# Rhizomatica/mercury

Hardware: AMD Instinct MI355X
Metric: RX frames/s (mode 8, max 50 LDPC iters) (higher is better)
Workload: dtype f64

## Files before the change

include/mercury_gpu.h:

```cpp
#ifndef MERCURY_GPU_H
#define MERCURY_GPU_H

#include <stddef.h>
#include <stdint.h>

#ifdef __cplusplus
extern "C" {
#endif

#define MGPU_OK 0
#define MGPU_ERR_ARG 1
#define MGPU_ERR_DEVICE 2
#define MGPU_ERR_TABLES 3
#define MGPU_ERR_UNSUPPORTED 4

#define MGPU_DEC_GBF 0
#define MGPU_DEC_SPA 1
#define MGPU_DEC_MINSUM 2
#define MGPU_DEC_SPA_FAST 3

#define MGPU_EST_ZF 0
#define MGPU_EST_LS 1

typedef struct mgpu_ctx mgpu_ctx;
// ... 130 lines not shown
    long long crc_ok_frames;
} mgpu_error_rate;
int mgpu_baseband_test_esn0(mgpu_ctx* ctx, const double* esn0_db, int npoints, long long frames_per_point, uint64_t seed, uint64_t frame0,
                            int channel, mgpu_error_rate* out);

int mgpu_passband_to_baseband(mgpu_ctx* ctx, const double* passband , int W, int in_size,
                              const double* carrier_hz , int filter, const int* start , int count,
                              int decimation, double* out_c128 );
int mgpu_time_sync_preamble(mgpu_ctx* ctx, const double* baseband_interp_c128 , int W, int size, int step,
                            int location_to_return, int nTrials_max, int* delay , double* correlation );
int mgpu_freq_sync(mgpu_ctx* ctx, const double* baseband_c128 , int W, int stride, double* freq_offset_hz );
int mgpu_time_sync_mfsk(mgpu_ctx* ctx, const double* baseband_interp_c128 , int W, int size, int search_start_symb,
                        int* delay );
int mgpu_detect_ack_pattern(mgpu_ctx* ctx, const double* baseband_interp_c128 , int W, int size, int pattern,
                            double* metric , int* matched );
int mgpu_detect_ack_pattern_from_passband(mgpu_ctx* ctx, const double* passband , int W, int size, double carrier_hz,
                                          int pattern, double* metric , int* matched );
int mgpu_last_sync_kernel_ms(mgpu_ctx* ctx, float* ms);

int mgpu_enable_timing(mgpu_ctx* ctx, int on);
int mgpu_kernel_ms_avg(mgpu_ctx* ctx, float ms[2], int* n_launches);
int mgpu_decoder_hard_frames(mgpu_ctx* ctx, long long* frames);
int mgpu_host_path_last(mgpu_ctx* ctx, int* chunk_frames, int* n_chunks, float* fill_ms, float* drain_ms, float* total_ms);
int mgpu_last_kernel_ms(mgpu_ctx* ctx, float ms[2]);

int mgpu_debug_mfsk_sync(mgpu_ctx* ctx, const double* energy, int W, int nslots, int size, const int* search_start, int variant, int* delay);
int mgpu_debug_p2b_variant(int variant);
int mgpu_debug_span_energy(mgpu_ctx* ctx, const double* bb, int W, int size, const int* wv, const int* off, int n, int len, int variant, double* sum,
                           int* cnt);
int mgpu_debug_spa_math(mgpu_ctx* ctx, const double* in, int n, double* tanh_out, double* atanh_out);
int mgpu_debug_select_peak(mgpu_ctx* ctx, const double* cand_vals, int n, int ncand_max, const int* ncand, const int* size, const int* loc, int step,
                           int nTrials_max, int* delay, double* corr);

int mgpu_debug_occupancy(mgpu_ctx* ctx, int which);

int mgpu_debug_tsync_metric(mgpu_ctx* ctx, const double* baseband_interp, int W, int size, int step, int variant, const int* start, const int* sub_size,
                            double* vals);

int mgpu_debug_glibc_trig(mgpu_ctx* ctx, const double* in, int n, double* atan_out, double* sin_out, double* cos_out);

#ifdef __cplusplus
}
#endif
#endif
```

mercury_amd/csrc/ctx.hpp:

```cpp
#pragma once
#include <hip/hip_runtime.h>

#include <functional>
#include <memory>
#include <stdexcept>
#include <string>
#include <type_traits>
#include <utility>
#include <vector>

#include <cmath>
#include "../../include/mercury_gpu.h"
#include "../../include/mercury_rxloop.h"
#include "../../include/mercury_channel.h"
#include "device_tables.h"
#include "tables.hpp"

extern "C" const unsigned char mgpu_ldpc_blob[];
extern "C" const unsigned long mgpu_ldpc_blob_size;

extern "C" size_t mgpu_frontend_lds_bytes(int G, int nPilots, int nBits, int threads);
extern "C" size_t mgpu_spa_lds_bytes(int E, int N);
extern "C" size_t mgpu_gbf_lds_bytes(int N);
extern "C" size_t mgpu_spa_fast_lds_bytes(int Sg, int N);
extern "C" size_t mgpu_txgen_lds_bytes(int G);

extern "C" __global__ void mgpu_frontend_kernel(MgpuDev, const double*, int, float*, float*, float*, double*, MgpuTapsDev);
extern "C" __global__ void mgpu_frontend_kernel_t1024(MgpuDev, const double*, int, float*, float*, float*, double*, MgpuTapsDev);
extern "C" __global__ void mgpu_mfsk_frontend_kernel_m32(MgpuDev, const double*, int, int, float*, float*, float*, MgpuTapsDev);
extern "C" __global__ void mgpu_mfsk_frontend_kernel_m16x2(MgpuDev, const double*, int, int, float*, float*, float*, MgpuTapsDev);
extern "C" int mgpu_mfsk_syms_per_block();
extern "C" __global__ void mgpu_slot_energy_kernel(const double*, int, int, int, const double*, double*);
extern "C" __global__ void mgpu_mfsk_sync_kernel(const double*, int, int, MgpuMfskSync, const int*, int*);
extern "C" __global__ void mgpu_zf_snr_kernel(MgpuDev, const uint8_t*, const double*, int, MgpuStatsDev*, double*);
extern "C" size_t mgpu_zfsnr_lds_bytes(int nData);
extern "C" __global__ void mgpu_p2b_kernel(const double*, int, const double*, const int*, int, int, int, const double*, int, double, double, double*, const int*, const double*, const int*, int);
extern "C" __global__ void mgpu_p2b_slide_d1_kernel(const double*, int, const double*, const int*, int, int, const double*, double, double, double*, const int*, const double*, const int*, int);
extern "C" __global__ void mgpu_p2b_slide_d4_kernel(const double*, int, const double*, const int*, int, int, const double*, double, double, double*, const int*, const double*, const int*, int);
extern "C" __global__ void mgpu_p2b_slide_d1_sincos_kernel(const double*, int, const double*, const int*, int, int, const double*, double, double, double*, const int*, const double*, const int*, int);
extern "C" __global__ void mgpu_p2b_slide_d4_sincos_kernel(const double*, int, const double*, const int*, int, int, const double*, double, double, double*, const int*, const double*, const int*, int);
struct MgpuKernelGeometry { int outputs_per_block, threads, lds_bytes; };
struct MgpuStreamGeometry { int step, ngi, nfft, pre, K, ring; };
extern "C" MgpuKernelGeometry mgpu_p2b_slide_geometry(int decim);
extern "C" __global__ void mgpu_tsync_metric_kernel(const double*, int, const int*, const int*, const int*, int, int, int, int, int, double*);
extern "C" __global__ void mgpu_tsync_metric_dense_kernel(const double*, int, const int*, const int*, const int*, int, int, int, int, int, double*);
extern "C" int mgpu_tsync_coarse_threads();
extern "C" __global__ void mgpu_tsync_metric_stream_kernel(const double*, int, const int*, const int*, const int*, int, double*, int, int, int);
extern "C" MgpuStreamGeometry mgpu_tsync_stream_geometry();
extern "C" __global__ void mgpu_tsync_metric_fine_kernel_r4(const double*, int, const int*, const int*, const int*, int, int, int, int, double*);
extern "C" __global__ void mgpu_tsync_metric_fine_kernel_r8(const double*, int, const int*, const int*, const int*, int, int, int, int, double*);
extern "C" MgpuKernelGeometry mgpu_tsync_fine_geometry(int R);
// ... 58 lines not shown
    using DevBuf::DevBuf;
    operator T*() const { return static_cast<T*>(p); }
};
template <typename H, hipError_t (*Destroy)(H)> struct Handle {
    H h = nullptr;
    Handle() = default;
    Handle(Handle&& o) noexcept { std::swap(h, o.h); }
    Handle& operator=(Handle&& o) noexcept { std::swap(h, o.h); return *this; }
    ~Handle() { if (h) (void)Destroy(h); }
    operator H() const { return h; }
};
using Stream = Handle<hipStream_t, hipStreamDestroy>;
using Event = Handle<hipEvent_t, hipEventDestroy>;
using GraphExec = Handle<hipGraphExec_t, hipGraphExecDestroy>;
using PinnedBuf = Handle<void*, hipHostFree>;

template <typename T>
DevArray<T> upload(const std::vector<T>& v) {
    DevArray<T> d(v.size() * sizeof(T) + 16);
    HIPCK(hipMemcpy(d.p, v.data(), v.size() * sizeof(T), hipMemcpyHostToDevice));
    return d;
}

struct Workspace;
struct TxState;
struct Release { void operator()(Workspace*) const; void operator()(TxState*) const; };

}
using namespace mgpu_detail;

struct mgpu_ctx {
    mgpu_config cfg{};
    mgpu::ModeTables tab;
    MgpuDev dev{};
    LdpcDev ldev{};
    std::vector<DevBuf> tables;
    std::string err;
    int max_batch = 0;
    int numa_node = -1;
    Stream stream;
    DevArray<double> d_baseband;
    DevArray<float> d_llr, d_variance, d_snrvar;
    DevArray<uint8_t> d_payload;
    DevArray<MgpuStatsDev> d_stats;
    DevArray<uint8_t> d_bits;
    DevArray<double> d_eqdata;
    double* d_fir[2] = {nullptr, nullptr};
    Event sync_ev[2];
    float last_sync_ms = -1.f;
    DevArray<int> d_iters;
    GraphExec one_frame_graph;
    DevArray<double> d_one_in;
    PinnedBuf h_one_in;
    PinnedBuf h_one_out;
    std::unique_ptr<Workspace, Release> rxloop_ws;
    int rxloop_ws_windows = 0;
    DevArray<double> rb_stage;
    DevArray<char> rb_compact;
    Stream rb_stream;
    DevArray<double> d_mix_cs;
    double mix_carrier = -1;
    size_t mix_count = 0;
    std::unique_ptr<TxState, Release> tx_state;
    std::vector<double> pre_eq;
    DevArray<double> d_pre_eq_buf;
    int pre_eq_version = 0;
    struct Pipe { Stream stream; Event done, copied; DevArray<double> d_in; };
    PinnedBuf h_out;
    static constexpr int kPipes = 2;
    Pipe pipe[kPipes];
    Event hp_ev[4];
    int hp_chunk = 0, hp_nchunks = 0;
    float hp_fill_ms = 0, hp_drain_ms = 0, hp_total_ms = 0;
    static constexpr int kEvRing = 64;
    Event ev[kEvRing][4];
    bool timing = false;
    int ev_count = 0;
    bool ev_fe[kEvRing]{};
    size_t lds_fe = 0, lds_dec = 0, lds_tx = 0;
    int fe_threads = 512;
    DecoderKernel spa_kernel = nullptr;
    int dec_threads = 1024;
    int wave_of_wgs = 0;

    template <typename T>
    T* keep(const std::vector<T>& v) { tables.push_back(upload(v)); return static_cast<T*>(tables.back().p); }
};


namespace mgpu_detail {

enum : unsigned { WS_FRONTEND = 1, WS_LLR = 2, WS_OUT = 4, WS_BITS = 8 };
void ensure_workspaces(mgpu_ctx* c, unsigned what);

constexpr int kMaxFramesPerLaunch = 1 << 21;
template <typename Fn> void for_frame_chunks(int F, Fn&& fn) {
    for (int off = 0; off < F; off += kMaxFramesPerLaunch) fn(off, F - off < kMaxFramesPerLaunch ? F - off : kMaxFramesPerLaunch);
}
template <typename T> T* at(T* p, size_t off) { return p ? p + off : nullptr; }

using FrontendKernel = void (*)(MgpuDev, const double*, int, float*, float*, float*, double*, MgpuTapsDev);
inline FrontendKernel fe_kernel(int threads) { return threads == 1024 ? mgpu_frontend_kernel_t1024 : mgpu_frontend_kernel; }

void launch_frontend(mgpu_ctx* c, const double* d_bb, int F, float* d_llr, float* d_var, float* d_snrvar, const MgpuTapsDev& taps,
                     hipStream_t s, int frame_stride = 0, int frame0 = 0);
void launch_zf_snr(mgpu_ctx* c, int F, const uint8_t* d_payload, MgpuStatsDev* d_stats, hipStream_t s, int frame0 = 0, double* d_var_out = nullptr);
void launch_decoder(mgpu_ctx* c, const float* d_llr, int F, uint8_t* d_bits, int* d_iters, uint8_t* d_payload, MgpuStatsDev* d_stats,
                    const float* d_var, const float* d_snrvar, hipStream_t s);
void launch_txgen(mgpu_ctx* c, uint64_t seed, uint64_t frame0, int F, double noise_amp, int channel, double* d_bb, uint8_t* d_payload, hipStream_t s,
                  const uint8_t* tx_payload = nullptr, int tx_stride = 0, const int* d_nbytes = nullptr);

int mfsk_sync_from_energies(const mgpu::ModeTables& t, const double* E, int nslots, int size, int search_start_symb);
void launch_mfsk_sync(mgpu_ctx* c, const double* d_energy, int W, int nslots, int size, const int* d_search_start, int* d_delay, hipStream_t s);
void launch_p2b(const double* passband, int in_size, const double* d_carrier, const int* d_start, int start_all, int count, int decim, const double* d_taps,
                int ntaps, double* out, const int* widx, const double* cs, const int* out_row, int row_by_launch, int nwin, hipStream_t s);
void select_peak(const double* cand_vals, int ncand, int step, int size, int location_to_return, int nTrials_max, int* delay, double* corr);

inline double moose_hz(double re, double im, double carrier_freq_width) {
    double theta = 0;
    if (re == 0) theta = M_PI / 2;
    else if (re > 0) theta = std::atan(im / re);
    else if (re < 0 && im >= 0) theta = std::atan(im / re) + M_PI;
    else if (re < 0 && im < 0) theta = std::atan(im / re) - M_PI;
    return (theta / M_PI) * carrier_freq_width;
}

const double* mixer_table(mgpu_ctx* c, double carrier_hz, size_t count, hipStream_t s);

// ... 82 lines not shown
```

mercury_amd/csrc/frontend.hip:

```cpp
#include <hip/hip_runtime.h>
#include <stdint.h>

#include "device_tables.h"
#include "fft256.h"
#include "fe_math.h"

namespace {

__device__ __attribute__((noinline)) c2 unit_phasor(c2 h) {
    const double th = get_angle(h);
    double s, c;
    gl_sincos(th, &s, &c);
    return {1 * c, 1 * s};
}

}

extern "C" __global__ void mgpu_glibc_trig_probe_kernel(const double* __restrict__ in, double* __restrict__ out_atan, double* __restrict__ out_sin,
                                                        double* __restrict__ out_cos, int n) {
    const int i = blockIdx.x * blockDim.x + threadIdx.x;
    if (i >= n) return;
    out_atan[i] = gl_atan(in[i]);
    double s, c;
    gl_sincos(in[i], &s, &c);
// ... 21 lines not shown
    c.rsz = (c.rsz + 15) & ~size_t(15);
    const size_t per_wave = size_t(FFT256_STRIDE) * 16, lds_cu = size_t(160) * 1024;
    const size_t aux0 = size_t((G + 15) & ~15) + 64, aux = aux0 > 2048 ? aux0 : 2048;
    const size_t fixed = size_t(16) * G + aux, need = size_t(16) * nPilots + c.rsz;
    const size_t minimal = fixed + (need > 4 * per_wave ? need : 4 * per_wave);
    const size_t block = 1280;
    const size_t overhead = 256;
    size_t wgs = lds_cu / ((minimal + overhead + block - 1) / block * block);
    const size_t cap = size_t(24 / FE_WAVES) > 0 ? size_t(24 / FE_WAVES) : 1;
    if (wgs > cap) wgs = cap;
    if (wgs < 1) wgs = 1;
    const size_t share = lds_cu / wgs / block * block;
    size_t w = share > fixed + overhead ? (share - overhead - fixed) / per_wave : 0;
    c.fft_waves = int(w < 4 ? 4 : (w > size_t(FE_WAVES) ? size_t(FE_WAVES) : w));
    c.work = need > c.fft_waves * per_wave ? need : c.fft_waves * per_wave;
    c.total = fixed + c.work;
    return c;
}
extern "C" size_t mgpu_frontend_lds_bytes(int G, int nPilots, int nBits, int threads) { return fe_carve(G, nPilots, nBits, threads / 64).total; }

template <int FE_THREADS>
__device__ __forceinline__ void fe_frame(const MgpuDev& T, const double* __restrict__ baseband, int F, float* __restrict__ llr_out,
                                         float* __restrict__ variance_out, float* __restrict__ snr_variance_out, double* __restrict__ eqdata_out,
                                         const MgpuTapsDev& taps) {
    constexpr int FE_WAVES = FE_THREADS / 64;
    extern __shared__ __attribute__((aligned(16))) unsigned char smem[];
    const int G = T.G, Nc = 50, Ns = T.Nsymb;
    const FeCarve carve = fe_carve(G, T.nPilots, T.nBits, FE_WAVES);
    c2* grid = reinterpret_cast<c2*>(smem);
    c2* Hp = grid + G;
    c2* fftb = Hp;
    double* red = reinterpret_cast<double*>(__builtin_assume_aligned(Hp + T.nPilots, 16));
    float* llr = reinterpret_cast<float*>(red);
    c2* yp = reinterpret_cast<c2*>(red);
    c2* tw = reinterpret_cast<c2*>(__builtin_assume_aligned(reinterpret_cast<unsigned char*>(Hp) + carve.work, 16));
    int8_t* type = reinterpret_cast<int8_t*>(tw);
    double* scal = reinterpret_cast<double*>(type + ((G + 15) & ~15));

    const int tid = threadIdx.x, lane = tid & 63, wave = tid >> 6;
    const int f = blockIdx.x;
    if (f >= F) return;
    const c2* bb = reinterpret_cast<const c2*>(baseband) + size_t(f) * T.frame_samples;
    const double boost = T.pilot_boost;
    int stamp_i = 0;
#define FE_STAMP() do { if (taps.cycles && f == (F >> 1) && tid == 0) taps.cycles[stamp_i] = __builtin_readcyclecounter(); ++stamp_i; } while (0)
    FE_STAMP();

    for (int i = tid; i < 128; i += FE_THREADS) tw[fft256_tw_slot(i)] = {T.twiddle[2 * i], T.twiddle[2 * i + 1]};
    __syncthreads();

    c2 n0 = {0, 0}, n1 = {0, 0}, n2 = {0, 0}, n3 = {0, 0};
    const Fft256CarrierLane fcl = fft256_carrier_lane(lane);
    const int nfw = carve.fft_waves;
    if (wave < nfw && wave < Ns) {
        const c2* in = bb + size_t(wave) * 272 + 16;
        n0 = in[lane]; n1 = in[lane + 64]; n2 = in[lane + 128]; n3 = in[lane + 192];
    }
    for (int s = wave; wave < nfw && s < Ns; s += nfw) {
        c2 r0 = n0, r1 = n1, r2 = n2, r3 = n3;
        if (s + nfw < Ns) {
            const c2* in = bb + size_t(s + nfw) * 272 + 16;
            n0 = in[lane]; n1 = in[lane + 64]; n2 = in[lane + 128]; n3 = in[lane + 192];
        }
        const c2 x = wave_fft256_carriers(r0, r1, r2, r3, fftb + wave * FFT256_STRIDE, tw, lane, fcl);
        if (fcl.col >= 0) grid[s * Nc + fcl.col] = {x.re / 256.0, x.im / 256.0};
    }
    __syncthreads();
    for (int i = tid; i < G; i += FE_THREADS) type[i] = T.cell_type[i] ? (T.pilot_val[i] < 0 ? int8_t(-1) : int8_t(1)) : int8_t(0);
    __syncthreads();

    FE_STAMP();
    if (T.agc) {
        for (int p = tid; p < T.nPilots; p += FE_THREADS) {
            const c2 y = grid[T.pilot_cell[p]];
            red[p] = sqrt(y.re * y.re + y.im * y.im);
        }
        __syncthreads();
        if (tid == 0) {
            double amp = serial_sum(red, T.nPilots);
            amp /= T.nPilots;
            scal[0] = boost / amp;
        }
        __syncthreads();
        const double agc = scal[0];
// ... 218 lines not shown
            const float D = float(dr * dr + di * di);
#pragma unroll
            for (int b = 0; b < 5; ++b) {
                if (b < bps) {
                    if ((j >> b) & 1) { if (D < d1[b]) d1[b] = D; }
                    else { if (D < d0[b]) d0[b] = D; }
                }
            }
        }
#pragma unroll
        for (int b = 0; b < 5; ++b)
            if (b < bps) llr[k * bps + (bps - 1 - b)] = inv_var * (d1[b] - d0[b]);
    }
    __syncthreads();
    if (taps.llr_demod) for (int i = tid; i < T.nBits; i += FE_THREADS) taps.llr_demod[size_t(f) * T.nBits + i] = llr[i];
    FE_STAMP();
    for (int p = tid; p < T.N; p += FE_THREADS) llr_out[size_t(f) * T.N + p] = llr[T.llr_src[p]];
    FE_STAMP();
#undef FE_STAMP
}

extern "C" __global__ __launch_bounds__(512, 6) void mgpu_frontend_kernel(
    MgpuDev T, const double* __restrict__ baseband, int F, float* __restrict__ llr_out,
    float* __restrict__ variance_out, float* __restrict__ snr_variance_out, double* __restrict__ eqdata_out, MgpuTapsDev taps) {
    fe_frame<512>(T, baseband, F, llr_out, variance_out, snr_variance_out, eqdata_out, taps);
}

extern "C" __global__ __launch_bounds__(1024, 4) void mgpu_frontend_kernel_t1024(
    MgpuDev T, const double* __restrict__ baseband, int F, float* __restrict__ llr_out,
    float* __restrict__ variance_out, float* __restrict__ snr_variance_out, double* __restrict__ eqdata_out, MgpuTapsDev taps) {
    fe_frame<1024>(T, baseband, F, llr_out, variance_out, snr_variance_out, eqdata_out, taps);
}
```

mercury_amd/csrc/launch.hip:

```cpp
#include <algorithm>
#include <atomic>
#include <cstdlib>

#include "ctx.hpp"

namespace mgpu_detail {

void launch_frontend(mgpu_ctx* c, const double* d_bb, int F, float* d_llr, float* d_var, float* d_snrvar,
                     const MgpuTapsDev& taps, hipStream_t s, int frame_stride, int frame0) {
    const int slot = c->ev_count % mgpu_ctx::kEvRing;
    const auto& t = c->tab;
    MgpuDev dev = c->dev;
    if (frame_stride > 0) dev.frame_samples = frame_stride;
    const size_t stride = size_t(dev.frame_samples);
    if (c->timing) { HIPCK(hipEventRecord(c->ev[slot][0], s)); c->ev_fe[slot] = true; }
    if (t.mfsk_M > 0) {
        const int per = mgpu_mfsk_syms_per_block(), chunks = (t.active_nsymb + per - 1) / per;
        if (!((t.mfsk_M == 32 && t.mfsk_nstreams == 1) || (t.mfsk_M == 16 && t.mfsk_nstreams == 2)) || t.mfsk_off[0] != 9 ||
            (t.mfsk_nstreams == 2 && t.mfsk_off[1] != 25) || t.Nc != 50)
            throw std::runtime_error("MFSK tone plan differs from the one the kernel is specialised for");
        const int max_frames = (1 << 23) / chunks;
        for (int off = 0; off < F; off += max_frames) {
            const int n = F - off < max_frames ? F - off : max_frames;
            if (off && (taps.grid || taps.llr_demod || taps.variance || taps.agc_gain))
                throw std::invalid_argument("stage taps are limited to one launch per call");
            hipLaunchKernelGGL(t.mfsk_M == 32 ? mgpu_mfsk_frontend_kernel_m32 : mgpu_mfsk_frontend_kernel_m16x2, dim3(unsigned(n) * chunks), dim3(256), 0, s, dev,
                               d_bb + size_t(off) * stride * 2, n, chunks, d_llr + size_t(off) * t.N, d_var + off, at(d_snrvar, off), taps);
            HIPCK(hipGetLastError());
        }
        if (c->timing) HIPCK(hipEventRecord(c->ev[slot][1], s));
        return;
    }
    for_frame_chunks(F, [&](int off, int n) {
        if (off && (taps.grid || taps.H || taps.eq || taps.syms || taps.llr_demod || taps.variance || taps.agc_gain || taps.mean_H))
            throw std::invalid_argument("stage taps are limited to 2^21 frames per call");
        hipLaunchKernelGGL(fe_kernel(c->fe_threads), dim3(n), dim3(c->fe_threads), c->lds_fe, s, dev, d_bb + size_t(off) * stride * 2, n,
                           d_llr + size_t(off) * t.N, d_var + off, at(d_snrvar, off), at<double>(c->d_eqdata, (size_t(frame0) + off) * t.nData * 2), taps);
        HIPCK(hipGetLastError());
    });
    if (c->timing) HIPCK(hipEventRecord(c->ev[slot][1], s));
}

void select_peak(const double* cand_vals, int ncand, int step, int size, int location_to_return, int nTrials_max, int* delay, double* corr) {
    if (location_to_return >= nTrials_max) location_to_return = nTrials_max - 1;
    const int j = location_to_return;
    auto original = [&](int i) { return (i % step == 0 && i / step < ncand) ? cand_vals[i / step] : 0.0; };
    double cur = j < size ? original(j) : 0.0;
    int loc = j;
    int p = j + 1;
    for (int k = (j + step) / step; k < ncand; ++k) {
        const int ci = k * step;
        if (ci <= j) continue;
        if (p < ci && cur < 0) { cur = 0.0; loc = p; }
        if (cand_vals[k] > cur) { cur = cand_vals[k]; loc = ci; }
        p = ci + 1;
    }
    if (p < size && cur < 0) { cur = 0.0; loc = p; }
    *delay = loc;
    *corr = cur;
}
// ... 167 lines not shown
```

mercury_amd/csrc/rx_batch.hip:

```cpp
#include <algorithm>
#include <cstdlib>
#include <cstring>

#include "ctx.hpp"

extern "C" {

int mgpu_enable_timing(mgpu_ctx* c, int on) {
    if (!c) return MGPU_ERR_ARG;
    c->timing = on != 0;
    c->ev_count = 0;
    for (auto& b : c->ev_fe) b = false;
    return MGPU_OK;
}

int mgpu_decoder_hard_frames(mgpu_ctx* c, long long* frames) {
    if (!c || !frames) return MGPU_ERR_ARG;
    return guard(c, [&] {
        HIPCK(hipStreamSynchronize(c->stream));
        unsigned long long v[64];
        HIPCK(hipMemcpy(v, c->ldev.hard_frames, sizeof(v), hipMemcpyDeviceToHost));
        long long sum = 0;
        for (unsigned long long x : v) sum += (long long)x;
        *frames = sum;
    });
}

// ... 165 lines not shown
                launch_zf_snr(c, 1, c->d_payload, c->d_stats, s);
                HIPCK(hipMemcpyAsync(c->h_one_out, c->d_payload, t.payload_stride, hipMemcpyDeviceToHost, s));
                HIPCK(hipMemcpyAsync(static_cast<char*>(c->h_one_out.h) + t.payload_stride, c->d_stats, sizeof(MgpuStatsDev), hipMemcpyDeviceToHost, s));
            } catch (...) {
                (void)hipStreamEndCapture(s, &graph);
                if (graph) (void)hipGraphDestroy(graph);
                throw;
            }
            HIPCK(hipStreamEndCapture(s, &graph));
            hipGraphExec_t exec = nullptr;
            const hipError_t e = hipGraphInstantiate(&exec, graph, nullptr, nullptr, 0);
            (void)hipGraphDestroy(graph);
            HIPCK(e);
            c->one_frame_graph.h = exec;
        }
        std::memcpy(c->h_one_in, bb, in_bytes);
        HIPCK(hipGraphLaunch(c->one_frame_graph, s));
        HIPCK(hipStreamSynchronize(s));
        if (payload) std::memcpy(payload, c->h_one_out, t.payload_stride);
        if (stats) std::memcpy(stats, static_cast<char*>(c->h_one_out.h) + t.payload_stride, sizeof(MgpuStatsDev));
    });
}

static void rx_batch_pipelined(mgpu_ctx* c, const double* bb, int F, uint8_t* payload, mgpu_frame_stats* stats) {
    const auto& t = c->tab;
    ensure_workspaces(c, WS_FRONTEND | WS_LLR | WS_OUT);
    const size_t frame_bytes = size_t(t.frame_samples) * 16;
    if (c->wave_of_wgs == 0) {
        int cus = 256;
        (void)hipDeviceGetAttribute(&cus, hipDeviceAttributeMultiprocessorCount, c->cfg.device);
        c->wave_of_wgs = 2 * (cus > 0 ? cus : 256);
    }
    const int wave_of_wgs = c->wave_of_wgs;
    int chunk = wave_of_wgs;
    while (size_t(chunk) * frame_bytes < (size_t(8) << 20)) chunk += wave_of_wgs;
    if (const char* e = std::getenv("MERCURY_RX_CHUNK")) chunk = std::max(1, std::atoi(e));
    chunk = std::min(chunk, F);
    for (auto& p : c->pipe) {
        if (!p.stream) HIPCK(hipStreamCreateWithFlags(&p.stream.h, hipStreamNonBlocking));
        if (!p.done) HIPCK(hipEventCreateWithFlags(&p.done.h, hipEventDisableTiming));
        if (!p.copied) HIPCK(hipEventCreateWithFlags(&p.copied.h, hipEventDisableTiming));
        if (p.d_in.capacity() < size_t(chunk) * frame_bytes) {
            HIPCK(hipStreamSynchronize(p.stream));
            p.d_in.grow(size_t(chunk) * frame_bytes);
        }
    }
    const size_t out_bytes = size_t(c->max_batch) * (t.payload_stride + sizeof(MgpuStatsDev));
    if (!c->h_out) HIPCK(host_alloc_on_node(&c->h_out.h, out_bytes + 16, c->numa_node));
    uint8_t* h_payload = static_cast<uint8_t*>(c->h_out.h);
    MgpuStatsDev* h_stats = reinterpret_cast<MgpuStatsDev*>(h_payload + ((size_t(c->max_batch) * t.payload_stride + 15) & ~size_t(15)));
    MgpuTapsDev none{};
    hipPointerAttribute_t attr{};
    const bool pinned = hipPointerGetAttributes(&attr, bb) == hipSuccess && attr.type == hipMemoryTypeHost;
    if (!pinned) (void)hipGetLastError();
    for (auto& e : c->hp_ev) if (!e) HIPCK(hipEventCreate(&e.h));
    const int nchunks = (F + chunk - 1) / chunk;
    int k = 0;
    for (int off = 0; off < F; off += chunk, ++k) {
        auto& p = c->pipe[k % mgpu_ctx::kPipes];
        hipStream_t cs = pinned ? c->pipe[0].stream : p.stream, ks = pinned ? c->pipe[1].stream : p.stream;
        const int n = std::min(chunk, F - off);
        if (pinned && k >= mgpu_ctx::kPipes) HIPCK(hipStreamWaitEvent(cs, p.done, 0));
        if (k == 0) HIPCK(hipEventRecord(c->hp_ev[0], cs));
        HIPCK(hipMemcpyAsync(p.d_in, reinterpret_cast<const char*>(bb) + size_t(off) * frame_bytes, size_t(n) * frame_bytes, hipMemcpyHostToDevice, cs));
        if (k == 0) HIPCK(hipEventRecord(c->hp_ev[1], cs));
        if (k == nchunks - 1) HIPCK(hipEventRecord(c->hp_ev[2], cs));
        if (pinned) {
            HIPCK(hipEventRecord(p.copied, cs));
            HIPCK(hipStreamWaitEvent(ks, p.copied, 0));
        }
        launch_frontend(c, p.d_in, n, c->d_llr + size_t(off) * t.N, c->d_variance + off, c->d_snrvar + off, none, ks, 0, off);
        if (pinned) HIPCK(hipEventRecord(p.done, ks));
        launch_decoder(c, c->d_llr + size_t(off) * t.N, n, nullptr, nullptr, c->d_payload + size_t(off) * t.payload_stride, c->d_stats + off,
                       c->d_variance + off, c->d_snrvar + off, ks);
        launch_zf_snr(c, n, c->d_payload + size_t(off) * t.payload_stride, c->d_stats + off, ks, off);
        if (payload) HIPCK(hipMemcpyAsync(h_payload + size_t(off) * t.payload_stride, c->d_payload + size_t(off) * t.payload_stride,
                                          size_t(n) * t.payload_stride, hipMemcpyDeviceToHost, ks));
        if (stats) HIPCK(hipMemcpyAsync(h_stats + off, c->d_stats + off, size_t(n) * sizeof(MgpuStatsDev), hipMemcpyDeviceToHost, ks));
        if (k == nchunks - 1) HIPCK(hipEventRecord(c->hp_ev[3], ks));
    }
    for (auto& p : c->pipe) HIPCK(hipStreamSynchronize(p.stream));
    c->hp_chunk = chunk; c->hp_nchunks = nchunks;
    (void)hipEventElapsedTime(&c->hp_fill_ms, c->hp_ev[0], c->hp_ev[1]);
    (void)hipEventElapsedTime(&c->hp_drain_ms, c->hp_ev[2], c->hp_ev[3]);
    (void)hipEventElapsedTime(&c->hp_total_ms, c->hp_ev[0], c->hp_ev[3]);
    if (payload) std::memcpy(payload, h_payload, size_t(F) * t.payload_stride);
    if (stats) std::memcpy(stats, h_stats, size_t(F) * sizeof(MgpuStatsDev));
}

int mgpu_host_path_last(mgpu_ctx* c, int* chunk_frames, int* n_chunks, float* fill_ms, float* drain_ms, float* total_ms) {
    if (!c) return MGPU_ERR_ARG;
    if (chunk_frames) *chunk_frames = c->hp_chunk;
    if (n_chunks) *n_chunks = c->hp_nchunks;
    if (fill_ms) *fill_ms = c->hp_fill_ms;
    if (drain_ms) *drain_ms = c->hp_drain_ms;
    if (total_ms) *total_ms = c->hp_total_ms;
    return MGPU_OK;
}

int mgpu_rx_batch(mgpu_ctx* c, const double* bb, int F, uint8_t* payload, mgpu_frame_stats* stats, float* llr_opt) {
    if (c && bb && F == 1 && !llr_opt && !c->timing && c->max_batch >= 1 && !std::getenv("MERCURY_NO_GRAPH"))
        return rx_one_frame(c, bb, payload, stats);
    if (c && bb && F > 1 && F <= c->max_batch && !llr_opt && !c->timing && !std::getenv("MERCURY_NO_PIPELINE"))
        return guard(c, [&] { rx_batch_pipelined(c, bb, F, payload, stats); });
    mgpu_stage_taps taps{};
    taps.llr_ldpc = llr_opt;
    return mgpu_rx_batch_taps(c, bb, F, payload, stats, llr_opt ? &taps : nullptr);
}

int mgpu_ldpc_batch(mgpu_ctx* c, const float* llr, int F, uint8_t* bits, int* iters) {
// ... 35 lines not shown
```

mercury_amd/physical_layer.py:

```python
import ctypes as C
import os

import numpy as np

HERE = os.path.dirname(os.path.abspath(__file__))
LIB_PATH = os.environ.get("MERCURY_GPU_LIB") or os.path.join(HERE, "libmercury_gpu.so")

DEC_GBF, DEC_SPA, DEC_MINSUM, DEC_SPA_FAST = 0, 1, 2, 3
EST_ZF, EST_LS = 0, 1


class Config(C.Structure):
    _fields_ = [("cfg", C.c_int), ("max_iters", C.c_int), ("decoder", C.c_int), ("agc", C.c_int),
                ("variance_source", C.c_int), ("device", C.c_int), ("max_batch", C.c_int),
                ("minsum_alpha", C.c_float), ("mfsk_ctrl_mode", C.c_int), ("test_puncture_nBits", C.c_int)]


INFO_FIELDS = ("cfg M bits_per_symbol K P N Nsymb Nc Nfft Ngi Nofdm nData nBits nPilots nVirtual nReal "
               "bit_blk tf_blk preamble_nsymb estimator amp_restore ls_window Cwidth Vwidth E "
               "payload_bytes payload_stride frame_samples mfsk_M mfsk_nStreams active_nsymb active_nbits").split()


class ExplicitParams(C.Structure):
    _fields_ = [("pilot_boost", C.c_float), ("ls_window", C.c_int), ("seeds_set", C.c_int), ("pilot_seed", C.c_uint),
# ... 47 lines not shown
        except Exception:
            pass
        lib = C.CDLL(LIB_PATH)
        lib.mgpu_last_error.restype = C.c_char_p
        lib.mgpu_last_error.argtypes = [C.c_void_p]
        lib.mgpu_create.argtypes = [C.POINTER(Config), C.POINTER(C.c_void_p)]
        lib.mgpu_txgen_dev.argtypes = [C.c_void_p, C.c_uint64, C.c_uint64, C.c_int, C.c_double, C.c_int,
                                       C.c_void_p, C.c_void_p, C.c_void_p]
        lib.mgpu_rx_batch_dev.argtypes = [C.c_void_p, C.c_void_p, C.c_int, C.c_void_p, C.c_void_p, C.c_void_p, C.c_void_p]
        lib.mgpu_frontend_dev.argtypes = [C.c_void_p, C.c_void_p, C.c_int, C.c_void_p, C.c_void_p, C.c_void_p]
        lib.mgpu_ldpc_batch_dev.argtypes = [C.c_void_p, C.c_void_p, C.c_int, C.c_void_p, C.c_void_p, C.c_void_p,
                                            C.c_void_p, C.c_void_p, C.c_void_p]
        lib.mgpu_destroy.argtypes = [C.c_void_p]
        _hf_argtypes(lib)
        _lib = lib
    return _lib


EXPORTED_SYMBOLS = [
    "mgpu_alloc_host", "mgpu_free_host", "mgpu_create", "mgpu_destroy", "mgpu_last_error", "mgpu_get_info", "mgpu_rx_batch", "mgpu_rx_batch_taps",
    "mgpu_host_libm_selfcheck", "mgpu_host_select_peak", "mgpu_host_fir_taps", "mgpu_host_preamble_carriers", "mgpu_host_mode_info", "mgpu_host_layout_stats",
    "mgpu_device_props_get", "mgpu_alloc_host_near", "mgpu_host_numa_node_of_pci", "mgpu_host_numa_cpus", "mgpu_pool_device_numa_node",
    "mgpu_ldpc_batch", "mgpu_ldpc_encode_batch", "mgpu_rx_batch_dev", "mgpu_frontend_dev", "mgpu_ldpc_batch_dev", "mgpu_txgen_dev",
    "mgpu_host_path_last", "mgpu_device_malloc", "mgpu_device_free", "mgpu_context_stream", "mgpu_synchronize", "mgpu_copy_to_host", "mgpu_copy_to_device",
    "mgpu_pool_rx_batch_dev", "mgpu_pool_ldpc_batch_dev", "mgpu_pool_txgen_dev",
    "mgpu_last_kernel_ms", "mgpu_kernel_ms_avg", "mgpu_decoder_hard_frames", "mgpu_enable_timing", "mgpu_debug_spa_math", "mgpu_debug_glibc_trig", "mgpu_debug_tsync_metric", "mgpu_debug_occupancy", "mgpu_debug_select_peak", "mgpu_debug_span_energy", "mgpu_debug_p2b_variant", "mgpu_debug_mfsk_sync", "mgpu_baseband_test_esn0", "mgpu_passband_test_esn0", "mgpu_passband_to_baseband", "mgpu_time_sync_preamble", "mgpu_freq_sync", "mgpu_last_sync_kernel_ms",
    "mgpu_time_sync_mfsk", "mgpu_detect_ack_pattern", "mgpu_detect_ack_pattern_from_passband",
    "mgpu_receive_buffer_nsymb", "mgpu_receive_byte_batch", "mgpu_receive_byte_batch_samples", "mgpu_measure_signal_only",
    "mgpu_host_pre_equalization_channel", "mgpu_context_pre_equalization_channel", "mgpu_set_pre_equalization_channel", "mgpu_transmit_bit_batch", "mgpu_transmit_frame_samples", "mgpu_transmit_byte_batch", "mgpu_transmit_byte_batch_dev", "mgpu_transmit_buffer", "mgpu_symbol_mod", "mgpu_generate_ack_pattern_passband",
    "mgpu_symbol_demod", "mgpu_automatic_gain_control", "mgpu_channel_estimator", "mgpu_restore_channel_amplitude", "mgpu_channel_equalizer",
    "mgpu_measure_variance", "mgpu_deframer", "mgpu_deinterleaver_c128", "mgpu_deinterleaver_f32", "mgpu_psk_demod",
    "mgpu_bit_energy_dispersal", "mgpu_bit_to_byte", "mgpu_crc16_modbus_rtu",
    "mgpu_shm_create", "mgpu_shm_connect", "mgpu_shm_close", "mgpu_shm_destroy", "mgpu_shm_used", "mgpu_shm_free", "mgpu_shm_capacity",
    "mgpu_shm_clear", "mgpu_shm_write", "mgpu_shm_read", "mgpu_shm_read_all", "mgpu_shm_publish_decoded",
    "mgpu_create_explicit", "mgpu_pool_create", "mgpu_pool_destroy", "mgpu_pool_size", "mgpu_pool_context", "mgpu_pool_last_error", "mgpu_pool_last_counters",
    "mgpu_pool_shard", "mgpu_pool_rx_batch", "mgpu_pool_ldpc_batch", "mgpu_pool_receive_byte_batch",
]


HF_MAX_PATHS, HF_SINUSOIDS = 4, 32
HF_PRESETS = {"awgn": 0, "good": 1, "moderate": 2, "poor": 3, "flutter": 4}
HF_CHANNEL_SYMBOLS = ["mgpu_hf_channel_preset", "mgpu_host_hilbert_taps", "mgpu_host_hf_channel_draws", "mgpu_host_hf_channel_taps",
                      "mgpu_hf_channel_apply", "mgpu_hf_channel_apply_dev", "mgpu_passband_test_esn0_hf", "mgpu_baseband_test_esn0_hf"]
HF_STREAM_SYMBOLS = ["mgpu_hf_stream_create", "mgpu_hf_stream_destroy", "mgpu_hf_stream_seek", "mgpu_hf_stream_latency", "mgpu_hf_stream_apply",
                     "mgpu_hf_stream_apply_dev", "mgpu_host_hf_stream_noise"]
HF_CHANNEL_SYMBOLS += HF_STREAM_SYMBOLS

# ... 479 lines not shown

    def debug_glibc_trig(self, x):
        xin = np.ascontiguousarray(x, np.float64)
        a, s, c = np.zeros_like(xin), np.zeros_like(xin), np.zeros_like(xin)
        self._ck(self.lib.mgpu_debug_glibc_trig(self.h, _ptr(xin), C.c_int(xin.size), _ptr(a), _ptr(s), _ptr(c)))
        return a, s, c

    def debug_spa_math(self, x):
        xin = np.ascontiguousarray(x, np.float64).ravel()
        t = np.zeros_like(xin)
        a = np.zeros_like(xin)
        self._ck(self.lib.mgpu_debug_spa_math(self.h, _ptr(xin), C.c_int(xin.size), _ptr(t), _ptr(a)))
        return t, a

    def enable_timing(self, on=True):
        self._ck(self.lib.mgpu_enable_timing(self.h, C.c_int(1 if on else 0)))

    def host_path_last(self):
        a, b = C.c_int(), C.c_int()
        f, d, t = C.c_float(), C.c_float(), C.c_float()
        self._ck(self.lib.mgpu_host_path_last(self.h, C.byref(a), C.byref(b), C.byref(f), C.byref(d), C.byref(t)))
        return {"chunk_frames": a.value, "n_chunks": b.value, "fill_ms": f.value, "drain_ms": d.value, "total_ms": t.value}

    def decoder_hard_frames(self):
        n = C.c_longlong(0)
        self._ck(self.lib.mgpu_decoder_hard_frames(self.h, C.byref(n)))
        return int(n.value)

    def kernel_ms_avg(self):
        ms = (C.c_float * 2)()
        n = C.c_int(0)
        self._ck(self.lib.mgpu_kernel_ms_avg(self.h, ms, C.byref(n)))
        return float(ms[0]), float(ms[1]), int(n.value)


POOL_MAX_DEVICES = 16


class ErrorRate(C.Structure):
    _fields_ = [("esn0_db", C.c_double), ("Frames_total", C.c_longlong), ("Error_frames_total", C.c_longlong), ("Bits_total", C.c_longlong),
                ("Error_bits_total", C.c_longlong), ("BER", C.c_double), ("FER", C.c_double), ("avg_iterations", C.c_double),
                ("crc_ok_frames", C.c_longlong)]


class PoolCounters(C.Structure):
    _fields_ = [("n_devices", C.c_int), ("frames", C.c_longlong), ("decoded", C.c_longlong), ("ldpc_iterations", C.c_longlong),
# ... 461 lines not shown
```

Measured before the change: 729,400.

## Pitch-strip cyclic prefix on H2D copy and overlap pageable copies via helper thread

The host-buffer RX pipeline now copies only the Nfft useful samples per OFDM symbol with a 2D strided memcpy, so the cyclic prefix never crosses the bus. The frontend kernel gains symbol pitch and offset parameters to read this packed layout. Copies move to a dedicated high-priority stream, and for pageable input a NUMA-bound helper thread issues them in parallel with kernel launches on the main thread. This adds threading, locking and schedule complexity, and the 2D copy may be less efficient than one flat copy.

```diff
diff --git a/include/mercury_gpu.h b/include/mercury_gpu.h
--- a/include/mercury_gpu.h
+++ b/include/mercury_gpu.h
@@ -176,6 +176,7 @@
 int mgpu_kernel_ms_avg(mgpu_ctx* ctx, float ms[2], int* n_launches);
 int mgpu_decoder_hard_frames(mgpu_ctx* ctx, long long* frames);
 int mgpu_host_path_last(mgpu_ctx* ctx, int* chunk_frames, int* n_chunks, float* fill_ms, float* drain_ms, float* total_ms);
+int mgpu_debug_host_path_schedule(int F, int chunk, int wave, int* out, int cap);
 int mgpu_last_kernel_ms(mgpu_ctx* ctx, float ms[2]);
 
 int mgpu_debug_mfsk_sync(mgpu_ctx* ctx, const double* energy, int W, int nslots, int size, const int* search_start, int variant, int* delay);
diff --git a/mercury_amd/csrc/ctx.hpp b/mercury_amd/csrc/ctx.hpp
--- a/mercury_amd/csrc/ctx.hpp
+++ b/mercury_amd/csrc/ctx.hpp
@@ -1,10 +1,13 @@
 #pragma once
 #include <hip/hip_runtime.h>
 
+#include <condition_variable>
 #include <functional>
 #include <memory>
+#include <mutex>
 #include <stdexcept>
 #include <string>
+#include <thread>
 #include <type_traits>
 #include <utility>
 #include <vector>
@@ -25,8 +28,8 @@
 extern "C" size_t mgpu_spa_fast_lds_bytes(int Sg, int N);
 extern "C" size_t mgpu_txgen_lds_bytes(int G);
 
-extern "C" __global__ void mgpu_frontend_kernel(MgpuDev, const double*, int, float*, float*, float*, double*, MgpuTapsDev);
-extern "C" __global__ void mgpu_frontend_kernel_t1024(MgpuDev, const double*, int, float*, float*, float*, double*, MgpuTapsDev);
+extern "C" __global__ void mgpu_frontend_kernel(MgpuDev, const double*, int, float*, float*, float*, double*, MgpuTapsDev, int, int);
+extern "C" __global__ void mgpu_frontend_kernel_t1024(MgpuDev, const double*, int, float*, float*, float*, double*, MgpuTapsDev, int, int);
 extern "C" __global__ void mgpu_mfsk_frontend_kernel_m32(MgpuDev, const double*, int, int, float*, float*, float*, MgpuTapsDev);
 extern "C" __global__ void mgpu_mfsk_frontend_kernel_m16x2(MgpuDev, const double*, int, int, float*, float*, float*, MgpuTapsDev);
 extern "C" int mgpu_mfsk_syms_per_block();
@@ -131,6 +134,23 @@
     return d;
 }
 
+class HelperThread {
+public:
+    HelperThread() = default;
+    HelperThread(const HelperThread&) = delete;
+    HelperThread& operator=(const HelperThread&) = delete;
+    ~HelperThread();
+    void run(int numa_node, std::function<void()> job);
+    void wait();
+private:
+    void loop(int numa_node);
+    std::thread th;
+    std::mutex m;
+    std::condition_variable cv;
+    std::function<void()> job;
+    bool has_job = false, busy = false, quit = false;
+};
+
 struct Workspace;
 struct TxState;
 struct Release { void operator()(Workspace*) const; void operator()(TxState*) const; };
@@ -174,10 +194,12 @@
     std::vector<double> pre_eq;
     DevArray<double> d_pre_eq_buf;
     int pre_eq_version = 0;
-    struct Pipe { Stream stream; Event done, copied; DevArray<double> d_in; };
+    struct Pipe { Stream stream; Event done, copied, ended; DevArray<double> d_in; };
     PinnedBuf h_out;
     static constexpr int kPipes = 2;
     Pipe pipe[kPipes];
+    Stream hp_copy;
+    HelperThread hp_helper;
     Event hp_ev[4];
     int hp_chunk = 0, hp_nchunks = 0;
     float hp_fill_ms = 0, hp_drain_ms = 0, hp_total_ms = 0;
@@ -208,11 +230,11 @@
 }
 template <typename T> T* at(T* p, size_t off) { return p ? p + off : nullptr; }
 
-using FrontendKernel = void (*)(MgpuDev, const double*, int, float*, float*, float*, double*, MgpuTapsDev);
+using FrontendKernel = void (*)(MgpuDev, const double*, int, float*, float*, float*, double*, MgpuTapsDev, int, int);
 inline FrontendKernel fe_kernel(int threads) { return threads == 1024 ? mgpu_frontend_kernel_t1024 : mgpu_frontend_kernel; }
 
 void launch_frontend(mgpu_ctx* c, const double* d_bb, int F, float* d_llr, float* d_var, float* d_snrvar, const MgpuTapsDev& taps,
-                     hipStream_t s, int frame_stride = 0, int frame0 = 0);
+                     hipStream_t s, int frame_stride = 0, int frame0 = 0, int sym_pitch = 0, int sym_first = 0);
 void launch_zf_snr(mgpu_ctx* c, int F, const uint8_t* d_payload, MgpuStatsDev* d_stats, hipStream_t s, int frame0 = 0, double* d_var_out = nullptr);
 void launch_decoder(mgpu_ctx* c, const float* d_llr, int F, uint8_t* d_bits, int* d_iters, uint8_t* d_payload, MgpuStatsDev* d_stats,
                     const float* d_var, const float* d_snrvar, hipStream_t s);
diff --git a/mercury_amd/csrc/frontend.hip b/mercury_amd/csrc/frontend.hip
--- a/mercury_amd/csrc/frontend.hip
+++ b/mercury_amd/csrc/frontend.hip
@@ -67,7 +67,7 @@
 template <int FE_THREADS>
 __device__ __forceinline__ void fe_frame(const MgpuDev& T, const double* __restrict__ baseband, int F, float* __restrict__ llr_out,
                                          float* __restrict__ variance_out, float* __restrict__ snr_variance_out, double* __restrict__ eqdata_out,
-                                         const MgpuTapsDev& taps) {
+                                         const MgpuTapsDev& taps, int sym_pitch, int sym_first) {
     constexpr int FE_WAVES = FE_THREADS / 64;
     extern __shared__ __attribute__((aligned(16))) unsigned char smem[];
     const int G = T.G, Nc = 50, Ns = T.Nsymb;
@@ -97,14 +97,16 @@
     c2 n0 = {0, 0}, n1 = {0, 0}, n2 = {0, 0}, n3 = {0, 0};
     const Fft256CarrierLane fcl = fft256_carrier_lane(lane);
     const int nfw = carve.fft_waves;
+    const int pitch = sym_pitch;
+    bb += sym_first;
     if (wave < nfw && wave < Ns) {
-        const c2* in = bb + size_t(wave) * 272 + 16;
+        const c2* in = bb + size_t(wave) * pitch;
         n0 = in[lane]; n1 = in[lane + 64]; n2 = in[lane + 128]; n3 = in[lane + 192];
     }
     for (int s = wave; wave < nfw && s < Ns; s += nfw) {
         c2 r0 = n0, r1 = n1, r2 = n2, r3 = n3;
         if (s + nfw < Ns) {
-            const c2* in = bb + size_t(s + nfw) * 272 + 16;
+            const c2* in = bb + size_t(s + nfw) * pitch;
             n0 = in[lane]; n1 = in[lane + 64]; n2 = in[lane + 128]; n3 = in[lane + 192];
         }
         const c2 x = wave_fft256_carriers(r0, r1, r2, r3, fftb + wave * FFT256_STRIDE, tw, lane, fcl);
@@ -369,12 +371,14 @@
 
 extern "C" __global__ __launch_bounds__(512, 6) void mgpu_frontend_kernel(
     MgpuDev T, const double* __restrict__ baseband, int F, float* __restrict__ llr_out,
-    float* __restrict__ variance_out, float* __restrict__ snr_variance_out, double* __restrict__ eqdata_out, MgpuTapsDev taps) {
-    fe_frame<512>(T, baseband, F, llr_out, variance_out, snr_variance_out, eqdata_out, taps);
+    float* __restrict__ variance_out, float* __restrict__ snr_variance_out, double* __restrict__ eqdata_out, MgpuTapsDev taps, int sym_pitch,
+    int sym_first) {
+    fe_frame<512>(T, baseband, F, llr_out, variance_out, snr_variance_out, eqdata_out, taps, sym_pitch, sym_first);
 }
 
 extern "C" __global__ __launch_bounds__(1024, 4) void mgpu_frontend_kernel_t1024(
     MgpuDev T, const double* __restrict__ baseband, int F, float* __restrict__ llr_out,
-    float* __restrict__ variance_out, float* __restrict__ snr_variance_out, double* __restrict__ eqdata_out, MgpuTapsDev taps) {
-    fe_frame<1024>(T, baseband, F, llr_out, variance_out, snr_variance_out, eqdata_out, taps);
-}
+    float* __restrict__ variance_out, float* __restrict__ snr_variance_out, double* __restrict__ eqdata_out, MgpuTapsDev taps, int sym_pitch,
+    int sym_first) {
+    fe_frame<1024>(T, baseband, F, llr_out, variance_out, snr_variance_out, eqdata_out, taps, sym_pitch, sym_first);
+}
diff --git a/mercury_amd/csrc/launch.hip b/mercury_amd/csrc/launch.hip
--- a/mercury_amd/csrc/launch.hip
+++ b/mercury_amd/csrc/launch.hip
@@ -7,11 +7,13 @@
 namespace mgpu_detail {
 
 void launch_frontend(mgpu_ctx* c, const double* d_bb, int F, float* d_llr, float* d_var, float* d_snrvar,
-                     const MgpuTapsDev& taps, hipStream_t s, int frame_stride, int frame0) {
+                     const MgpuTapsDev& taps, hipStream_t s, int frame_stride, int frame0, int sym_pitch, int sym_first) {
     const int slot = c->ev_count % mgpu_ctx::kEvRing;
     const auto& t = c->tab;
     MgpuDev dev = c->dev;
     if (frame_stride > 0) dev.frame_samples = frame_stride;
+    if (sym_pitch > 0) need(t.mfsk_M == 0 && sym_first >= 0 && sym_pitch >= t.Nfft, "symbol layout: OFDM modes only, at least Nfft samples per symbol");
+    else { sym_pitch = t.Nofdm; sym_first = t.Ngi; }
     const size_t stride = size_t(dev.frame_samples);
     if (c->timing) { HIPCK(hipEventRecord(c->ev[slot][0], s)); c->ev_fe[slot] = true; }
     if (t.mfsk_M > 0) {
@@ -35,7 +37,7 @@
         if (off && (taps.grid || taps.H || taps.eq || taps.syms || taps.llr_demod || taps.variance || taps.agc_gain || taps.mean_H))
             throw std::invalid_argument("stage taps are limited to 2^21 frames per call");
         hipLaunchKernelGGL(fe_kernel(c->fe_threads), dim3(n), dim3(c->fe_threads), c->lds_fe, s, dev, d_bb + size_t(off) * stride * 2, n,
-                           d_llr + size_t(off) * t.N, d_var + off, at(d_snrvar, off), at<double>(c->d_eqdata, (size_t(frame0) + off) * t.nData * 2), taps);
+                           d_llr + size_t(off) * t.N, d_var + off, at(d_snrvar, off), at<double>(c->d_eqdata, (size_t(frame0) + off) * t.nData * 2), taps, sym_pitch, sym_first);
         HIPCK(hipGetLastError());
     });
     if (c->timing) HIPCK(hipEventRecord(c->ev[slot][1], s));
diff --git a/mercury_amd/csrc/rx_batch.hip b/mercury_amd/csrc/rx_batch.hip
--- a/mercury_amd/csrc/rx_batch.hip
+++ b/mercury_amd/csrc/rx_batch.hip
@@ -3,6 +3,7 @@
 #include <cstring>
 
 #include "ctx.hpp"
+#include "numa.hpp"
 
 extern "C" {
 
@@ -214,7 +215,85 @@
     });
 }
 
-static void rx_batch_pipelined(mgpu_ctx* c, const double* bb, int F, uint8_t* payload, mgpu_frame_stats* stats) {
+
+}
+
+namespace mgpu_detail {
+
+HelperThread::~HelperThread() {
+    {
+        std::lock_guard<std::mutex> lk(m);
+        quit = true;
+    }
+    cv.notify_all();
+    if (th.joinable()) th.join();
+}
+void HelperThread::loop(int numa_node) {
+    const char* e = std::getenv("MERCURY_POOL_AFFINITY");
+    if (!(e && e[0] == '0')) (void)mgpu_numa::bind_thread_to_node(numa_node);
+    std::unique_lock<std::mutex> lk(m);
+    for (;;) {
+        cv.wait(lk, [&] { return has_job || quit; });
+        if (quit) return;
+        std::function<void()> fn = std::move(job);
+        has_job = false;
+        lk.unlock();
+        fn();
+        lk.lock();
+        busy = false;
+        cv.notify_all();
+    }
+}
+void HelperThread::run(int numa_node, std::function<void()> fn) {
+    std::unique_lock<std::mutex> lk(m);
+    cv.wait(lk, [&] { return !busy; });
+    job = std::move(fn); has_job = true; busy = true;
+    if (!th.joinable()) th = std::thread([this, numa_node] { loop(numa_node); });
+    cv.notify_all();
+}
+void HelperThread::wait() {
+    std::unique_lock<std::mutex> lk(m);
+    cv.wait(lk, [&] { return !busy; });
+}
+
+}
+
+namespace {
+
+std::vector<int> taper(int F, int chunk, int tail) {
+    std::vector<int> out;
+    if (F <= 0) return out;
+    chunk = std::max(1, std::min(chunk, F));
+    tail = std::max(1, tail);
+    int rest = F;
+    if (chunk <= tail) {
+        for (; rest > 0; rest -= chunk) out.push_back(std::min(chunk, rest));
+        return out;
+    }
+    for (; rest > 2 * chunk; rest -= chunk) out.push_back(chunk);
+    while (rest > tail) {
+        const int p = std::min(chunk, (rest + 1) / 2);
+        out.push_back(p);
+        rest -= p;
+    }
+    if (rest > 0) out.push_back(rest);
+    return out;
+}
+
+std::vector<int> host_path_schedule(int F, int chunk, int wave) {
+    (void)wave;
+    if (const char* e = std::getenv("MERCURY_RX_CHUNK")) chunk = std::max(1, std::atoi(e));
+    int tail = chunk;
+    if (const char* e = std::getenv("MERCURY_RX_TAIL")) tail = std::max(1, std::atoi(e));
+    return taper(F, chunk, tail);
+}
+
+int env_switch(const char* name) {
+    const char* e = std::getenv(name);
+    return e && e[0] ? (e[0] != '0') : -1;
+}
+
+void rx_batch_pipelined(mgpu_ctx* c, const double* bb, int F, uint8_t* payload, mgpu_frame_stats* stats) {
     const auto& t = c->tab;
     ensure_workspaces(c, WS_FRONTEND | WS_LLR | WS_OUT);
     const size_t frame_bytes = size_t(t.frame_samples) * 16;
@@ -226,58 +305,177 @@
     const int wave_of_wgs = c->wave_of_wgs;
     int chunk = wave_of_wgs;
     while (size_t(chunk) * frame_bytes < (size_t(8) << 20)) chunk += wave_of_wgs;
-    if (const char* e = std::getenv("MERCURY_RX_CHUNK")) chunk = std::max(1, std::atoi(e));
-    chunk = std::min(chunk, F);
+    const std::vector<int> pieces = host_path_schedule(F, chunk, wave_of_wgs);
+    const int npieces = int(pieces.size());
+    chunk = *std::max_element(pieces.begin(), pieces.end());
+
+    hipPointerAttribute_t attr{};
+    const bool pinned = hipPointerGetAttributes(&attr, bb) == hipSuccess && attr.type == hipMemoryTypeHost;
+    if (!pinned) (void)hipGetLastError();
+    const bool ofdm = t.mfsk_M == 0 && t.Nofdm == t.Ngi + t.Nfft && t.frame_samples == t.Nsymb * t.Nofdm;
+    const int want_pitched = env_switch("MERCURY_RX_PITCHED");
+    const bool pitched = ofdm && want_pitched != 0;
+    const int want_helper = env_switch("MERCURY_RX_HELPER");
+    const bool helper = npieces > 1 && (want_helper >= 0 ? want_helper != 0 : !pinned);
+    const size_t dev_frame_samples = pitched ? size_t(t.Nsymb) * t.Nfft : size_t(t.frame_samples);
+
+    if (!c->hp_copy) {
+        int least = 0, greatest = 0;
+        HIPCK(hipDeviceGetStreamPriorityRange(&least, &greatest));
+        HIPCK(hipStreamCreateWithPriority(&c->hp_copy.h, hipStreamNonBlocking, greatest));
+    }
+    const hipStream_t copy_stream = c->hp_copy;
     for (auto& p : c->pipe) {
         if (!p.stream) HIPCK(hipStreamCreateWithFlags(&p.stream.h, hipStreamNonBlocking));
         if (!p.done) HIPCK(hipEventCreateWithFlags(&p.done.h, hipEventDisableTiming));
         if (!p.copied) HIPCK(hipEventCreateWithFlags(&p.copied.h, hipEventDisableTiming));
-        if (p.d_in.capacity() < size_t(chunk) * frame_bytes) {
+        if (!p.ended) HIPCK(hipEventCreateWithFlags(&p.ended.h, hipEventDisableTiming));
+        if (p.d_in.capacity() < size_t(chunk) * dev_frame_samples * 16) {
             HIPCK(hipStreamSynchronize(p.stream));
-            p.d_in.grow(size_t(chunk) * frame_bytes);
+            p.d_in.grow(size_t(chunk) * dev_frame_samples * 16);
         }
     }
     const size_t out_bytes = size_t(c->max_batch) * (t.payload_stride + sizeof(MgpuStatsDev));
     if (!c->h_out) HIPCK(host_alloc_on_node(&c->h_out.h, out_bytes + 16, c->numa_node));
     uint8_t* h_payload = static_cast<uint8_t*>(c->h_out.h);
     MgpuStatsDev* h_stats = reinterpret_cast<MgpuStatsDev*>(h_payload + ((size_t(c->max_batch) * t.payload_stride + 15) & ~size_t(15)));
+    for (auto& e : c->hp_ev) if (!e) HIPCK(hipEventCreate(&e.h));
+    std::vector<int> first(npieces);
+    for (int k = 0, off = 0; k < npieces; off += pieces[k], ++k) first[k] = off;
+
+    auto queue_copy = [&](int k) {
+        auto& p = c->pipe[k % mgpu_ctx::kPipes];
+        const int off = first[k], n = pieces[k];
+        const hipStream_t cs = (pinned || helper) ? copy_stream : p.stream;
+        if (k >= mgpu_ctx::kPipes) HIPCK(hipStreamWaitEvent(cs, p.done, 0));
+        if (k == 0) HIPCK(hipEventRecord(c->hp_ev[0], cs));
+        const char* src = reinterpret_cast<const char*>(bb) + size_t(off) * frame_bytes;
+        if (pitched)
+            HIPCK(hipMemcpy2DAsync(p.d_in, size_t(t.Nfft) * 16, src + size_t(t.Ngi) * 16, size_t(t.Nofdm) * 16, size_t(t.Nfft) * 16,
+                                   size_t(n) * t.Nsymb, hipMemcpyHostToDevice, cs));
+        else
+            HIPCK(hipMemcpyAsync(p.d_in, src, size_t(n) * frame_bytes, hipMemcpyHostToDevice, cs));
+        if (k == 0) HIPCK(hipEventRecord(c->hp_ev[1], cs));
+        if (k == npieces - 1) HIPCK(hipEventRecord(c->hp_ev[2], cs));
+        HIPCK(hipEventRecord(p.copied, cs));
+    };
     MgpuTapsDev none{};
-    hipPointerAttribute_t attr{};
-    const bool pinned = hipPointerGetAttributes(&attr, bb) == hipSuccess && attr.type == hipMemoryTypeHost;
-    if (!pinned) (void)hipGetLastError();
-    for (auto& e : c->hp_ev) if (!e) HIPCK(hipEventCreate(&e.h));
-    const int nchunks = (F + chunk - 1) / chunk;
-    int k = 0;
-    for (int off = 0; off < F; off += chunk, ++k) {
+    auto queue_kernels = [&](int k) {
         auto& p = c->pipe[k % mgpu_ctx::kPipes];
-        hipStream_t cs = pinned ? c->pipe[0].stream : p.stream, ks = pinned ? c->pipe[1].stream : p.stream;
-        const int n = std::min(chunk, F - off);
-        if (pinned && k >= mgpu_ctx::kPipes) HIPCK(hipStreamWaitEvent(cs, p.done, 0));
-        if (k == 0) HIPCK(hipEventRecord(c->hp_ev[0], cs));
-        HIPCK(hipMemcpyAsync(p.d_in, reinterpret_cast<const char*>(bb) + size_t(off) * frame_bytes, size_t(n) * frame_bytes, hipMemcpyHostToDevice, cs));
-        if (k == 0) HIPCK(hipEventRecord(c->hp_ev[1], cs));
-        if (k == nchunks - 1) HIPCK(hipEventRecord(c->hp_ev[2], cs));
-        if (pinned) {
-            HIPCK(hipEventRecord(p.copied, cs));
-            HIPCK(hipStreamWaitEvent(ks, p.copied, 0));
-        }
-        launch_frontend(c, p.d_in, n, c->d_llr + size_t(off) * t.N, c->d_variance + off, c->d_snrvar + off, none, ks, 0, off);
-        if (pinned) HIPCK(hipEventRecord(p.done, ks));
+        const hipStream_t ks = p.stream;
+        const int off = first[k], n = pieces[k];
+        HIPCK(hipStreamWaitEvent(ks, p.copied, 0));
+        launch_frontend(c, p.d_in, n, c->d_llr + size_t(off) * t.N, c->d_variance + off, c->d_snrvar + off, none, ks,
+                        pitched ? int(dev_frame_samples) : 0, off, pitched ? t.Nfft : 0, 0);
+        HIPCK(hipEventRecord(p.done, ks));
         launch_decoder(c, c->d_llr + size_t(off) * t.N, n, nullptr, nullptr, c->d_payload + size_t(off) * t.payload_stride, c->d_stats + off,
                        c->d_variance + off, c->d_snrvar + off, ks);
         launch_zf_snr(c, n, c->d_payload + size_t(off) * t.payload_stride, c->d_stats + off, ks, off);
         if (payload) HIPCK(hipMemcpyAsync(h_payload + size_t(off) * t.payload_stride, c->d_payload + size_t(off) * t.payload_stride,
                                           size_t(n) * t.payload_stride, hipMemcpyDeviceToHost, ks));
         if (stats) HIPCK(hipMemcpyAsync(h_stats + off, c->d_stats + off, size_t(n) * sizeof(MgpuStatsDev), hipMemcpyDeviceToHost, ks));
-        if (k == nchunks - 1) HIPCK(hipEventRecord(c->hp_ev[3], ks));
-    }
-    for (auto& p : c->pipe) HIPCK(hipStreamSynchronize(p.stream));
-    c->hp_chunk = chunk; c->hp_nchunks = nchunks;
+        if (k == npieces - 1) {
+            if (npieces > 1) {
+                auto& q = c->pipe[(k + 1) % mgpu_ctx::kPipes];
+                HIPCK(hipEventRecord(q.ended, q.stream));
+                HIPCK(hipStreamWaitEvent(ks, q.ended, 0));
+            }
+            HIPCK(hipEventRecord(c->hp_ev[3], ks));
+        }
+    };
+    auto settle = [&] {
+        c->hp_helper.wait();
+        hipError_t e = hipStreamSynchronize(copy_stream);
+        for (auto& p : c->pipe) { const hipError_t e2 = hipStreamSynchronize(p.stream); if (e == hipSuccess) e = e2; }
+        return e;
+    };
+
+    if (!helper) {
+        try {
+            for (int k = 0; k < npieces; ++k) { queue_copy(k); queue_kernels(k); }
+        } catch (...) {
+            (void)settle();
+            throw;
+        }
+    } else {
+        std::mutex m;
+        std::condition_variable cv;
+        int copies = 0, kernels = 0;
+        bool stop = false;
+        std::string copy_error;
+        c->hp_helper.run(c->numa_node, [&] {
+            std::string err;
+            try {
+                HIPCK(hipSetDevice(c->cfg.device));
+                for (int k = 0; k < npieces; ++k) {
+                    {
+                        std::unique_lock<std::mutex> lk(m);
+                        cv.wait(lk, [&] { return stop || kernels > k - mgpu_ctx::kPipes; });
+                        if (stop) break;
+                    }
+                    queue_copy(k);
+                    {
+                        std::lock_guard<std::mutex> lk(m);
+                        copies = k + 1;
+                    }
+                    cv.notify_all();
+                }
+            } catch (const std::exception& e) {
+                err = e.what();
+            }
+            if (!err.empty()) {
+                std::lock_guard<std::mutex> lk(m);
+                copy_error = err; stop = true;
+            }
+            cv.notify_all();
+        });
+        try {
+            for (int k = 0; k < npieces; ++k) {
+                {
+                    std::unique_lock<std::mutex> lk(m);
+                    cv.wait(lk, [&] { return stop || copies > k; });
+                    if (stop) break;
+                }
+                queue_kernels(k);
+                {
+                    std::lock_guard<std::mutex> lk(m);
+                    kernels = k + 1;
+                }
+                cv.notify_all();
+            }
+        } catch (...) {
+            {
+                std::lock_guard<std::mutex> lk(m);
+                stop = true;
+            }
+            cv.notify_all();
+            (void)settle();
+            throw;
+        }
+        c->hp_helper.wait();
+        if (!copy_error.empty()) {
+            (void)settle();
+            throw HipError("input copy of the host-buffer pipeline: " + copy_error);
+        }
+    }
+    HIPCK(settle());
+    c->hp_chunk = chunk; c->hp_nchunks = npieces;
     (void)hipEventElapsedTime(&c->hp_fill_ms, c->hp_ev[0], c->hp_ev[1]);
     (void)hipEventElapsedTime(&c->hp_drain_ms, c->hp_ev[2], c->hp_ev[3]);
     (void)hipEventElapsedTime(&c->hp_total_ms, c->hp_ev[0], c->hp_ev[3]);
     if (payload) std::memcpy(payload, h_payload, size_t(F) * t.payload_stride);
     if (stats) std::memcpy(stats, h_stats, size_t(F) * sizeof(MgpuStatsDev));
+}
+
+}
+
+extern "C" {
+
+int mgpu_debug_host_path_schedule(int F, int chunk, int wave, int* out, int cap) {
+    if (F < 0 || chunk < 1 || wave < 1 || (cap > 0 && !out)) return -1;
+    const std::vector<int> pieces = host_path_schedule(F, chunk, wave);
+    for (int i = 0; i < int(pieces.size()) && i < cap; ++i) out[i] = pieces[i];
+    return int(pieces.size());
 }
 
 int mgpu_host_path_last(mgpu_ctx* c, int* chunk_frames, int* n_chunks, float* fill_ms, float* drain_ms, float* total_ms) {
diff --git a/mercury_amd/physical_layer.py b/mercury_amd/physical_layer.py
--- a/mercury_amd/physical_layer.py
+++ b/mercury_amd/physical_layer.py
@@ -93,7 +93,7 @@
     "mgpu_host_libm_selfcheck", "mgpu_host_select_peak", "mgpu_host_fir_taps", "mgpu_host_preamble_carriers", "mgpu_host_mode_info", "mgpu_host_layout_stats",
     "mgpu_device_props_get", "mgpu_alloc_host_near", "mgpu_host_numa_node_of_pci", "mgpu_host_numa_cpus", "mgpu_pool_device_numa_node",
     "mgpu_ldpc_batch", "mgpu_ldpc_encode_batch", "mgpu_rx_batch_dev", "mgpu_frontend_dev", "mgpu_ldpc_batch_dev", "mgpu_txgen_dev",
-    "mgpu_host_path_last", "mgpu_device_malloc", "mgpu_device_free", "mgpu_context_stream", "mgpu_synchronize", "mgpu_copy_to_host", "mgpu_copy_to_device",
+    "mgpu_host_path_last", "mgpu_debug_host_path_schedule", "mgpu_device_malloc", "mgpu_device_free", "mgpu_context_stream", "mgpu_synchronize", "mgpu_copy_to_host", "mgpu_copy_to_device",
     "mgpu_pool_rx_batch_dev", "mgpu_pool_ldpc_batch_dev", "mgpu_pool_txgen_dev",
     "mgpu_last_kernel_ms", "mgpu_kernel_ms_avg", "mgpu_decoder_hard_frames", "mgpu_enable_timing", "mgpu_debug_spa_math", "mgpu_debug_glibc_trig", "mgpu_debug_tsync_metric", "mgpu_debug_occupancy", "mgpu_debug_select_peak", "mgpu_debug_span_energy", "mgpu_debug_p2b_variant", "mgpu_debug_mfsk_sync", "mgpu_baseband_test_esn0", "mgpu_passband_test_esn0", "mgpu_passband_to_baseband", "mgpu_time_sync_preamble", "mgpu_freq_sync", "mgpu_last_sync_kernel_ms",
     "mgpu_time_sync_mfsk", "mgpu_detect_ack_pattern", "mgpu_detect_ack_pattern_from_passband",
@@ -619,6 +619,15 @@
         self._ck(self.lib.mgpu_host_path_last(self.h, C.byref(a), C.byref(b), C.byref(f), C.byref(d), C.byref(t)))
         return {"chunk_frames": a.value, "n_chunks": b.value, "fill_ms": f.value, "drain_ms": d.value, "total_ms": t.value}
 
+    @staticmethod
+    def host_path_schedule(F, chunk, wave=512):
+        lib = load_library()
+        out = (C.c_int * max(1, F))()
+        n = lib.mgpu_debug_host_path_schedule(C.c_int(F), C.c_int(chunk), C.c_int(wave), out, C.c_int(len(out)))
+        if n < 0:
+            raise ValueError("mgpu_debug_host_path_schedule: bad argument")
+        return [int(out[i]) for i in range(n)]
+
     def decoder_hard_frames(self):
         n = C.c_longlong(0)
         self._ck(self.lib.mgpu_decoder_hard_frames(self.h, C.byref(n)))
```

New measurement: 731,200, median of 3. No clear change (+0.3%).
